# ksaintmarc/Montecarlo-PathTracing

Hardware: AMD Instinct MI355X
Metric: Msamples/s (W×H×spp/s) + achieved HBM GB/s, 1080p scene6, 1/2/4/8 GPU (higher is better)
Workload: dtype f32

## Files before the change

### montecarlo-pathtracing_amd/csrc/mcpt_capi.hip

```cpp
#include <algorithm>
#include <cmath>
#include <cstdio>
#include <cstring>
#include <new>

#include "mcpt_ctx.h"
#include "mcpt_math.h"

namespace plan = mcpt::plan;
static_assert(plan::kCandLane == MCPT_TRAVERSAL_LANE && plan::kCandWave == MCPT_TRAVERSAL_WAVE &&
              plan::kCandStream == MCPT_TRAVERSAL_STREAM, "candidates 1..3 are the traversal modes");

static thread_local char g_last_error[256] = "";
static thread_local char g_detail[320] = "";
static thread_local int g_last_status = 0;
static thread_local bool g_fresh = false;

int set_err(int status, const char* what, hipError_t e) {
  if (e != hipSuccess)
    std::snprintf(g_last_error, sizeof(g_last_error), "%s: %s", what, hipGetErrorString(e));
  else
    std::snprintf(g_last_error, sizeof(g_last_error), "%s", what);
  g_last_status = status;
  g_fresh = true;
// ... 822 lines not shown
  p.split_of = L.d_split_of;
  p.split_pass = L.d_split_pass;
  p.split_max = plan::kSplitMax;
  if (p.item_perm) p.split_n = L.d_split_n;
  if (steal) {
    OK_OR_RETURN(ensure_lane_bytes(c, L.d_steal, L.steal_bytes,
                                   sizeof(float) * 3 * (size_t)items * mcpt::kPassChunk * mcpt::kTileThreads));
    p.steal_vals = L.d_steal;
  }
  return MCPT_OK;
}

static int sort_order(mcpt_ctx* c, mcpt_ctx::Lane& L, hipStream_t ws, const plan::Items& it, const mcpt::RenderParams& p) {
  size_t tmp = L.sort_tmp_bytes;
  HIP_OR_RETURN(mcpt_order_items(L.d_item_cost, L.d_cost_sorted, L.d_item_iota, L.d_item_perm, (int)it.items,
                                 L.d_sort_tmp, &tmp, ws));
  if (c->n_meshes > 0)
    HIP_OR_RETURN(mcpt_split_count(L.d_cost_sorted, (int)it.items, 20 / (p.tile_w / 8) * c->n_cu, plan::kSplitMax,
                                   L.d_split_n, c->d_events + kDebugSplitSlot, ws));
  std::copy(it.key, it.key + 8, L.order_key);
  L.order_valid = true;
  L.order_age = 0;
  return MCPT_OK;
}

static int launch(mcpt_ctx* c, const float* invPV, const float* invV, int first_pass, int n_passes, float date,
                  int bounces, float refract_ind, int variant, bool count, unsigned long long* events) {
  OK_OR_RETURN(check_renderable(c, invPV && invV && n_passes >= 0 && variant >= 0 && variant <= 2, "mcpt_render"));
  invalidate_planes(c);
  HIP_OR_RETURN(hipSetDevice(c->device));
  mcpt::RenderParams p;
  scene_params(c, invPV, invV, p);
  plan::Tuner& tuner = c->tuner;
  HIP_OR_RETURN(collect_tuning(c, (tuner.pending_other_shape(p.n_local_px, n_passes) || count) ? 0 : 1));
  p.n_tiles = ((c->W + p.tile_w - 1) / p.tile_w) * ((c->n_local_rows + mcpt::kTileH - 1) / mcpt::kTileH);
  const long long total_seg = plan::pass_segments(first_pass, n_passes);
  tuner.deep_auto = c->depth >= 8;
  const int cand = count ? (c->traversal == MCPT_TRAVERSAL_AUTO ? MCPT_TRAVERSAL_LANE : c->traversal)
                         : resolve_candidate(c, total_seg);
  const bool stream = cand == plan::kCandStream && stream_applies(c, variant, bounces, count);
  c->stream_iters = 0;
  p.wave_traversal = (cand == MCPT_TRAVERSAL_WAVE) ? 1 : 0;
  p.walk_exit = plan::cand_walk_exit(cand, c->walk_exit, c->n_meshes, c->depth);
  p.leaf_batch = plan::cand_leaf_batch(cand, c->leaf_batch, c->depth);
  p.walk_min_done = plan::cand_deep_knobs(cand) ? plan::kDeepMinDone : 1;
  if (const int md = env_int("MCPT_WALK_MIN_DONE", 0); md > 0) p.walk_min_done = md;
  p.seg_per_item = plan::resolved_seg_per_item(cand, env_int("MCPT_SEG_PER_ITEM", 0));
  pass_params(first_pass, n_passes, date, bounces, refract_ind, variant, p);
  const bool steal = env_int("MCPT_STEAL", 1) != 0;
  plan::LimitsIn lin;
  lin.n_local_px = p.n_local_px; lin.n_tiles = p.n_tiles; lin.tile_w = p.tile_w; lin.seg_per_item = p.seg_per_item;
  lin.n_cu = c->n_cu; lin.partial_budget = c->partial_budget; lin.mesh = c->n_meshes > 0;
  lin.wave_traversal = p.wave_traversal != 0; lin.steal = steal;
  const plan::Limits lim = plan::limits(lin);
  if (lim.too_large) return set_err(MCPT_ERR_INVALID_ARG, "render target too large for one launch");
  const bool split = plan::pass_split(lim, p.n_tiles, n_passes, total_seg, c->n_cu, stream, env_int("MCPT_PASS_SPLIT", -1));
  p.pass_split = split ? 1 : 0;
  if (split) p.seg_per_item = 1;
  const int n_sub = plan::count_sub_launches(first_pass, n_passes, lim.max_seg, split);
  const size_t seg_bytes = (size_t)p.n_local_px * 3 * sizeof(float);
  const int slot = (c->ring_pos + 1) % kTimingRing;
  HIP_OR_RETURN(ensure_events(c, slot, std::max(n_sub, 1)));
  const bool lanes_ok = tuner.overlap != 0 && !count && !stream && schedule_settled(c);
  if (count) HIP_OR_RETURN(hipMemsetAsync(c->d_events, 0, sizeof(unsigned long long) * mcpt::EV_COUNT, c->stream));
  if (n_sub == 0) {
    for (int i = 0; i < kEvPerSub; ++i) HIP_OR_RETURN(hipEventRecord(ev_at(c, slot, 0, i), c->stream));
    c->ring_lane[slot][0] = 0;
  }
  plan::ItemsIn in;
  in.n_tiles = p.n_tiles; in.seg_per_item = p.seg_per_item; in.walk_exit = p.walk_exit; in.bounces = bounces;
  in.variant = variant; in.tile_w = p.tile_w; in.n_cu = c->n_cu; in.wave_traversal = p.wave_traversal != 0;
  in.pass_split = split; in.mesh = c->n_meshes > 0;
  in.orderable = !count && !stream && env_int("MCPT_ITEM_ORDER", 1) != 0;
  in.split_items_on = env_int("MCPT_SPLIT_ITEMS", 1) != 0;
  in.tail_pieces_on = env_int("MCPT_TAIL_PIECES", 1) != 0;
  int k = 0;
  for (long long lo = first_pass, end = (long long)first_pass + n_passes; lo < end; lo = in.sub.end(), ++k) {
    in.sub = plan::next_sub_launch(lo, end, lim.max_seg, split);
    const plan::Items it = plan::items(in);
    p.first_pass = in.sub.first_pass; p.n_passes = in.sub.n_passes; p.n_segments = in.sub.n_segments;
    p.item_perm = nullptr;
    p.item_cost = nullptr;
    p.split_n = nullptr; p.split_of = nullptr; p.split_pass = nullptr; p.split_max = 0;
    p.steal_vals = nullptr;
    p.n_items = (int)it.items;
    p.tail_m = 0;
#ifdef MCPT_CHECKED
    p.check_inject = env_int("MCPT_CHECKED_INJECT", 0);
#endif
    const int li = c->next_lane;
    c->next_lane ^= 1;
    mcpt_ctx::Lane& L = c->lanes[li];
    const bool lane = lanes_ok && p.n_segments > 1;
    hipStream_t ws = lane ? L.stream : c->stream;
    if (p.n_segments > 1) OK_OR_RETURN(ensure_lane_bytes(c, L.d_partial, L.partial_bytes, (size_t)p.n_segments * seg_bytes));
    p.partial = L.d_partial;
    if (it.order) HIP_OR_RETURN(ensure_item_order(c, L, it.items));
    if (lane) HIP_OR_RETURN(hipStreamWaitEvent(L.stream, lane_freed(c, L), 0));
    if (it.order) OK_OR_RETURN(prepare_order(c, li, ws, in, it, p));
    if (it.split_items) OK_OR_RETURN(prepare_split_items(c, L, ws, it.items, steal, p));
    const bool period = lane && c->prev_lane >= 0 && c->prev_lane != li;
    HIP_OR_RETURN(hipEventRecord(ev_at(c, slot, k, 0), period ? c->lanes[c->prev_lane].stream : ws));
    if (lane) HIP_OR_RETURN(hipEventRecord(ev_at(c, slot, k, 3), ws));
    c->ring_lane[slot][k] = lane;
    if (stream) {
      OK_OR_RETURN(stream_run(c, p));
    } else {
      HIP_OR_RETURN(mcpt_launch_render(p, count, ws));
    }
    HIP_OR_RETURN(hipEventRecord(ev_at(c, slot, k, 1), ws));
    if (lane) {
      HIP_OR_RETURN(hipStreamWaitEvent(c->stream, ev_at(c, slot, k, 1), 0));
      if (period) HIP_OR_RETURN(hipStreamWaitEvent(c->stream, ev_at(c, slot, k, 0), 0));
    }
    HIP_OR_RETURN(mcpt_launch_combine(p, c->stream));
    HIP_OR_RETURN(hipEventRecord(ev_at(c, slot, k, 2), c->stream));
    if (it.order && (!p.item_perm || ++L.order_age >= plan::kOrderRefresh)) OK_OR_RETURN(sort_order(c, L, ws, it, p));
    if (lane) {
      HIP_OR_RETURN(hipEventRecord(L.tail, L.stream));
      HIP_OR_RETURN(hipStreamWaitEvent(c->stream, L.tail, 0));
      HIP_OR_RETURN(hipEventRecord(L.freed, c->stream));
    }
    L.freed_stale = !lane;
    c->prev_lane = lane ? li : -1;
#ifdef MCPT_CHECKED
    OK_OR_RETURN(checked_sub_launch(c, k, n_sub, p));
#endif
  }
  if (!count && c->traversal == MCPT_TRAVERSAL_AUTO)
    tuner.issue(cand, (double)p.n_local_px * n_passes, p.n_local_px, n_passes, total_seg, slot);
  c->n_sub = std::max(n_sub, 1);
  c->ring_pos = slot;
  c->ring_n_sub[slot] = c->n_sub;
  c->n_timed++;
  c->pass_split = split ? 1 : 0;
  c->timed = true;
  c->pass_count += n_passes;
  if (c->ad_on && n_passes > 0)
    HIP_OR_RETURN(mcpt_launch_adaptive_add_passes(adaptive_target(c), nullptr, 0, n_passes, c->stream));
  if (c->stats_on && n_passes > 0) HIP_OR_RETURN(stats_batch(c, n_passes));
  if (count) {
    unsigned long long h[mcpt::EV_COUNT];
    HIP_OR_RETURN(hipMemcpyAsync(h, c->d_events, sizeof(h), hipMemcpyDeviceToHost, c->stream));
    HIP_OR_RETURN(hipStreamSynchronize(c->stream));
    for (int e = 0; e < mcpt::EV_COUNT; ++e) events[e] += h[e];
  }
  return MCPT_OK;
}

int mcpt_render(mcpt_ctx* c, const float* invPV, const float* invV, int first_pass, int n_passes, float date,
                int bounces, float refract_ind, int variant) {
  return launch(c, invPV, invV, first_pass, n_passes, date, bounces, refract_ind, variant, false, nullptr);
}
// ... 321 lines not shown
```

### montecarlo-pathtracing_amd/csrc/mcpt_internal.h

```cpp
#pragma once
#include <hip/hip_runtime.h>
#include <stdint.h>
#include "mcpt_plan.h"

int mcpt_err_bare(int status);

namespace mcpt {

enum { EV_NODE = 0, EV_LEAF, EV_PRIM, EV_CAND, EV_GEOM, EV_COLMAT, EV_SAMPLE, EV_TRAV, EV_MESH, EV_TRI, EV_MGEOM,
       EV_COUNT };

constexpr int kEventBytes[EV_COUNT] = {
    48,
    4,
    16 + 64,
    64,
    64,
    32,
    24,
    0,
    12 + 64 + 64,
    12 + 36,
    12 + 72 + 64,
};
// ... 194 lines not shown
                                hipStream_t stream);
hipError_t mcpt_launch_variance_init(const mcpt::CountSource* counts, const float* accum, float4* out,
                                     const float4* guide, const float2* emap, int W, int H, int pass_count,
                                     hipStream_t stream);
namespace mcpt {
struct TemporalParams {
  const float* accum;
  const float2* emap;
  const float4* guide;
  const float4* hc_in;
  const int* hl_in;
  const float4* hg_in;
  float4* hc_out;
  int* hl_out;
  float4* hg_out;
  unsigned long long* rec;
  int W, H;
  float nb;
  int max_history;
  float plane_tol;
  int empty;
  float M[16];
};
}
hipError_t mcpt_launch_temporal(const mcpt::TemporalParams& p, hipStream_t stream);
hipError_t mcpt_launch_temporal_init(const float4* hc, float4* out, const float4* guide, int W, int H,
                                     hipStream_t stream);
hipError_t mcpt_launch_pack_counted(const mcpt::CountSource& src, int n_rows, const float* accum, void* out,
                                    hipStream_t stream);
hipError_t mcpt_launch_load_rows_counted(const void* src, const int* src_row, int W, int H, float* accum, int* plane,
                                         hipStream_t stream);
hipError_t mcpt_launch_load_rows_error_map(const void* src, const int* src_row, int W, int H, float2* plane,
                                           hipStream_t stream);
hipError_t mcpt_iota(int* a, int n, hipStream_t stream);
hipError_t mcpt_split_count(const unsigned* cost_sorted, int n, int capacity, int split_max, int* out,
                            unsigned long long* dbg, hipStream_t stream);
constexpr int kDebugSplitSlot = 63;
constexpr int kDebugStealSlot = 62;

namespace mcpt {
constexpr int kCheckedCountSlot = 60, kCheckedSiteSlot = 61;
enum CheckSite {
  CK_SPLIT_N = 1,
  CK_PERM_SPLIT,
  CK_PERM_TAIL,
  CK_PERM_HEAD,
  CK_ITEM,
  CK_SPLIT_OF,
  CK_SPLIT_PASS,
  CK_SEGMENT,
  CK_PIXEL,
  CK_COMBINE_SPLIT,
  CK_LIST,
  CK_COUNT
};
#ifdef MCPT_CHECKED
constexpr bool kChecked = true;
__device__ inline bool idx_ok(unsigned long long* ev, int site, long long i, long long n) {
  if (i >= 0 && i < n) return true;
  if (ev) {
    atomicAdd(ev + kCheckedCountSlot, 1ull);
    atomicCAS(ev + kCheckedSiteSlot, 0ull, ((unsigned long long)site << 48) | ((unsigned long long)i & 0xffffffffffffull));
  }
  return false;
}
#else
constexpr bool kChecked = false;
__device__ __forceinline__ bool idx_ok(unsigned long long*, int, long long, long long) { return true; }
#endif
}
hipError_t mcpt_order_items(const unsigned* cost, unsigned* cost_sorted, const int* iota, int* perm, int n,
                            void* tmp, size_t* tmp_bytes, hipStream_t stream);
hipError_t mcpt_launch_stream_init(const mcpt::StreamParams& q, hipStream_t stream);
hipError_t mcpt_launch_stream_iter(const mcpt::StreamParams& q, int n_cu, bool lds_nodes, hipStream_t stream);
bool mcpt_stream_lds_nodes_fit(int depth);
```

### montecarlo-pathtracing_amd/csrc/mcpt_kernel.hip

```cpp
#include <hip/hip_runtime.h>
#include <stdint.h>
#include "mcpt_device.h"

constexpr int kMinWaves = 7;


namespace mcpt {

constexpr int kMinWavesMesh = 5;
constexpr int kMinWavesL2 = 7;
template <bool COUNT, bool WAVE, bool MESH, bool LDSS, bool SUSPEND, int TW, bool LIST = false>
__global__ __launch_bounds__(TW * kTileH, MESH && !WAVE ? kMinWavesMesh
                                           : (!WAVE && !LDSS ? kMinWavesL2 : kMinWaves)) void render_kernel(
    RenderParams p) {
  constexpr int TT = TW * kTileH;
  const int tid = threadIdx.x;
  const int lane = tid & 63, wave = tid >> 6;
  constexpr bool kSplit = MESH && !WAVE && !COUNT && !LIST;
  int item, piece = -1, sj = -1;
  if constexpr (kChecked) {
    if (p.check_inject) (void)idx_ok(p.events, CK_PERM_HEAD, blockIdx.x, p.n_items);
  }
  if constexpr (kSplit) {
    const int b = blockIdx.x;
    int sn = (p.item_perm && p.split_n) ? *p.split_n : 0;
    if (!idx_ok(p.events, CK_SPLIT_N, sn, (long long)p.split_max + 1)) sn = 0;
    if (b < sn * kSplitPieces) {
      sj = b / kSplitPieces;
      piece = b - sj * kSplitPieces;
      if (!idx_ok(p.events, CK_PERM_SPLIT, sj, p.n_items)) return;
      item = p.item_perm[sj];
    } else {
      const int r = sn + (b - sn * kSplitPieces);
      if (r >= p.n_items) return;
      item = p.item_perm ? p.item_perm[r] : r;
    }
  }
  int seg_only = -1;
  if constexpr (!kSplit) {
    const int b = blockIdx.x;
    const int head = p.tail_m > 0 ? p.n_items - p.tail_m : p.n_items;
    if (b >= head && p.tail_m > 0) {
      const int q = b - head, j = q / p.seg_per_item;
      if (!idx_ok(p.events, CK_PERM_TAIL, head + j, p.n_items)) return;
      item = p.item_perm[head + j];
      seg_only = q - j * p.seg_per_item;
    } else {
      if (!idx_ok(p.events, CK_PERM_HEAD, b, p.n_items)) return;
      item = p.item_perm ? p.item_perm[b] : b;
    }
  }
  if (!idx_ok(p.events, CK_ITEM, item, p.n_items)) return;
  const unsigned long long t_item0 = __builtin_amdgcn_s_memrealtime();
#ifdef MCPT_BLOCKTIMES
  const unsigned long long bt0 = __builtin_amdgcn_s_memrealtime();
#endif

  const int K = p.seg_per_item > 1 ? p.seg_per_item : 1;
  const int n_groups = (p.n_segments + K - 1) / K;
  const int tile = item / n_groups;
  int seg_lo = (item % n_groups) * K;
  int seg_n = min(K, p.n_segments - seg_lo);
  if (seg_only >= 0) {
    if (seg_only >= seg_n) return;
    seg_lo += seg_only;
    seg_n = 1;
  }
  int seg = seg_lo;
  const int tiles_x = (p.W + TW - 1) / TW;
  int bx0 = (tile % tiles_x) * TW + (wave % (TW / 8)) * 8;
  int by0 = (tile / tiles_x) * kTileH + (wave / (TW / 8)) * 8;
  bool listed = true;
  if constexpr (LIST) {
    static_assert(!COUNT && !WAVE, "LIST: the per-lane render kernels only");
    const long long li = (long long)tile * (TW / 8) + wave;
    int n_list = p.n_list;
    if (n_list < 0) {
      n_list = min(max(p.list[p.n_blocks], 0), -n_list);
      if ((long long)tile * (TW / 8) >= n_list) return;
    }
    listed = li < n_list && idx_ok(p.events, CK_LIST, li, p.n_blocks);
    const int blk = listed ? p.list[li] : 0;
    listed = listed && idx_ok(p.events, CK_LIST, blk, p.n_blocks);
    bx0 = (blk % p.blocks_x) * 8;
    by0 = (blk / p.blocks_x) * 8;
  }
  const int x = bx0 + (lane & 7);
  const int lr = by0 + (lane >> 3);
  const bool live = x < p.W && lr < p.n_local_rows && listed;
  const int cbase = floordiv(p.first_pass - 1, kPassChunk);
  const int c0 = cbase + seg_lo;
  int pass_begin = max(p.first_pass, c0 * kPassChunk + 1);
  int pass_end = min(p.first_pass + p.n_passes, (c0 + 1) * kPassChunk + 1);
  if (p.pass_split) {
    pass_begin = p.first_pass + seg_lo;
    pass_end = pass_begin + 1;
  }
  const int seg_first = pass_begin;
  int b1 = 0;
  if (kSplit && piece >= 0) {
    const int n = pass_end - pass_begin;
    b1 = pass_begin + n / kSplitPieces;
    const int lo = pass_begin + (piece * n) / kSplitPieces, hi = pass_begin + ((piece + 1) * n) / kSplitPieces;
    pass_begin = lo;
    pass_end = hi;
    if (piece == 0 && tid == 0 && idx_ok(p.events, CK_SPLIT_OF, item, p.n_items)) p.split_of[item] = sj;
  }
  const int y = live ? p.rows[lr] : 0;

  SceneT<MESH, LDSS> s{p.nodes, p.leaves, p.ptype, p.prims, p.depth, p.minfo, p.mpairs, p.mleaftris, p.mtris,
                       p.mverts, p.mnorms, p.flat_face};
  if constexpr (LDSS) {
    extern __shared__ float4 s_scene[];
    const int n_nodes = (2 << p.depth) - 1, n_leaves = 1 << p.depth;
    const int n4 = 3 * n_nodes + 8 * p.n_prims;
    for (int i = tid; i < n4; i += TT) s_scene[i] = i < 3 * n_nodes ? p.nodes[i] : p.prims[i - 3 * n_nodes];
    int* s_int = (int*)(s_scene + n4);
    for (int i = tid; i < n_leaves + p.n_prims; i += TT)
      s_int[i] = i < n_leaves ? p.leaves[i] : p.ptype[i - n_leaves];
    __syncthreads();
    s.nodes = s_scene;
    s.prims = s_scene + 3 * n_nodes;
    s.leaves = s_int;
    s.ptype = s_int + n_leaves;
  }
  static_assert(!kSplit || TT == 64, "pass stealing: one wave per workgroup (LDS order, unit mapping)");
  const bool steal = kSplit && p.steal_vals != nullptr;
  __shared__ int s_claim;
  __shared__ unsigned s_stolen;
  if constexpr (kSplit) {
    if (steal) {
      if (tid == 0) { s_claim = TT; s_stolen = 0u; }
      __syncthreads();
    }
  }
  Ev<COUNT> ev;
  ev.init();
#ifdef MCPT_LANESTATS
  for (int k = lane; k < LS_COUNT; k += 64) ls_row()[k] = 0u;
  __builtin_amdgcn_wave_barrier();
  if (!live) return;
#else
  if (!live) return;
#endif

  const float u = ((float)x + 0.5f) / (float)p.W;
  const float v = ((float)y + 0.5f) / (float)p.H;
  constexpr bool kPixLds = !LDSS || (MESH && !WAVE);
  constexpr bool kPxLds = kPixLds && MESH;
  constexpr bool kIorConst = kPixLds;
  __shared__ float s_pix[kPxLds ? 21 : (kPixLds ? 20 : 18)][TT];
  __shared__ int s_hit0[TT];
  const f3 Dcam0 = camera_dir(p, u, v);
  s_pix[0][tid] = Dcam0.x; s_pix[1][tid] = Dcam0.y; s_pix[2][tid] = Dcam0.z;
  if constexpr (kPixLds) {
    s_pix[18][tid] = u; s_pix[19][tid] = v;
    if constexpr (kPxLds) s_pix[20][tid] = __int_as_float(lr * p.W + x);
  }
  int pj = tid;
  auto pix_seed = [&](int ps) {
    if constexpr (kPixLds) return seed_for(s_pix[18][pj], s_pix[19][pj], ps, p.date);
    else return seed_for(((float)x + 0.5f) / (float)p.W, ((float)y + 0.5f) / (float)p.H, ps, p.date);
  };
  s_pix[12][tid] = 0.0f; s_pix[13][tid] = 0.0f; s_pix[14][tid] = 0.0f;
  const f3 Ocam = mk(p.ox, p.oy, p.oz);


  const float ior = p.ior;
  const int B = p.bounces;
  int pass = pass_begin;
  Rng rng = seed_for(u, v, pass, p.date);
  f3 O = Ocam, D = Dcam0, att = mk(0.8f, 0.8f, 0.8f), total = mk(0.0f, 0.0f, 0.0f);
  f3 N = mk(0.0f, 0.0f, 0.0f), P = mk(0.0f, 0.0f, 0.0f);
  int bounce = 0, phase = 0;
  Hit h;
  h.pl = mk(0.0f, 0.0f, 0.0f); h.dist = kFLTMAX; h.clear(); h.tri = 0;
  h.cull2 = 0.0;

  int key0 = -1;
  f3 N0 = N, P0 = P;
  const bool run = !(p.variant == 0 && B <= 0);
#ifdef MCPT_STAMPS
  unsigned long long st_k0 = __builtin_amdgcn_s_memtime(), st_t = 0, st_s = 0, st_it = 0;
#endif
  if (!COUNT && run) {
    traverse<COUNT, WAVE, SUSPEND && !LDSS && !MESH>(s, Ocam, Dcam0, h, ev);
    key0 = hit_key(h);
    if (h.hit()) geom_info<COUNT>(s, h, N0, P0, ev);
  }
  s_pix[3][tid] = N0.x; s_pix[4][tid] = N0.y; s_pix[5][tid] = N0.z;
  s_pix[6][tid] = P0.x; s_pix[7][tid] = P0.y; s_pix[8][tid] = P0.z;
  s_hit0[tid] = key0;

#ifdef MCPT_STAMPS
  const unsigned long long st_p = __builtin_amdgcn_s_memtime() - st_k0;
#endif
  auto flush_sum = [&]() {
    if (kSplit && (piece > 0 || steal)) return;
    size_t px;
    if constexpr (kPxLds) {
      px = (size_t)(unsigned)__float_as_int(s_pix[20][tid]);
    } else {
      int lrow = lr, col = x;
      asm volatile("" : "+v"(lrow), "+v"(col));
      px = (size_t)lrow * p.W + col;
    }
    if (!idx_ok(p.events, CK_PIXEL, (long long)px, p.n_local_px)) return;
    if (p.n_segments == 1) {
      float* accp = p.accum + px * 3;
      accp[0] = accp[0] + s_pix[12][tid]; accp[1] = accp[1] + s_pix[13][tid]; accp[2] = accp[2] + s_pix[14][tid];
    } else {
      if (!idx_ok(p.events, CK_SEGMENT, seg, p.n_segments)) return;
      float* part = p.partial + ((size_t)seg * p.n_local_px + px) * 3;
      part[0] = s_pix[12][tid]; part[1] = s_pix[13][tid]; part[2] = s_pix[14][tid];
    }
  };
  auto add_pass = [&](f3 v) {
    if (kSplit && steal) {
      if constexpr (kChecked) {
        if (!idx_ok(p.events, CK_SPLIT_PASS, pass - seg_first, kPassChunk) || !idx_ok(p.events, CK_SPLIT_PASS, pj, kTileThreads))
          return;
      }
      float* q = p.steal_vals + (((size_t)item * kPassChunk + (pass - seg_first)) * kTileThreads + pj) * 3;
      q[0] = v.x; q[1] = v.y; q[2] = v.z;
      return;
    }
    if (kSplit && piece > 0) {
      if constexpr (kChecked) {
        if (!idx_ok(p.events, CK_SPLIT_PASS, sj, p.split_max) || !idx_ok(p.events, CK_SPLIT_PASS, pass - b1, kPassChunk) ||
            !idx_ok(p.events, CK_SPLIT_PASS, tid, kTileThreads))
          return;
      }
      float* q = p.split_pass + (((size_t)sj * kPassChunk + (pass - b1)) * kTileThreads + tid) * 3;
      q[0] = v.x; q[1] = v.y; q[2] = v.z;
    } else {
      s_pix[12][tid] = s_pix[12][tid] + v.x;
      s_pix[13][tid] = s_pix[13][tid] + v.y;
      s_pix[14][tid] = s_pix[14][tid] + v.z;
    }
  };
  const int steal_n = pass_end - pass_begin;
  auto steal_next = [&]() {
    for (;;) {
      const int u = atomicAdd(&s_claim, 1);
      if (u >= TT * steal_n) { pass = pass_end; return; }
      const int t = u % TT;
      const int xt = bx0 + (t & 7), lt = by0 + (t >> 3);
      if (xt < p.W && lt < p.n_local_rows) {
        pj = t; pass = pass_begin + u / TT;
        if (t != tid) atomicAdd(&s_stolen, 1u);
        return;
      }
    }
  };
  auto next_chunk = [&]() {
    if (kSplit && steal) {
      steal_next();
      return;
    }
    if (pass >= pass_end) {
      flush_sum();
      if (seg + 1 < seg_lo + seg_n) {
        seg++;
        const int c = c0 + (seg - seg_lo);
        pass = c * kPassChunk + 1;
        pass_end = min(p.first_pass + p.n_passes, (c + 1) * kPassChunk + 1);
        s_pix[12][tid] = 0.0f; s_pix[13][tid] = 0.0f; s_pix[14][tid] = 0.0f;
      }
    }
  };
  Walk walk;
  walk.invD = mk(0.0f, 0.0f, 0.0f); walk.node = 0; walk.level = 0; walk.pending = 0; walk.mpf = 0;
  bool walking = false;
#ifdef MCPT_LANESTATS
  ls_add(LS_WAVES, 1u);
#endif
  while (pass < pass_end) {
#ifdef MCPT_STAMPS
    const unsigned long long st_a = __builtin_amdgcn_s_memtime();
    st_it++;
#endif
#ifdef MCPT_LANESTATS
    ls_add(LS_ROUNDS, 1u);
    ls_add(LS_ROUND_LN, ls_pop(true));
#endif
    bool done = false;
    f3 res = mk(0.0f, 0.0f, 0.0f);
    bool first = !COUNT && bounce == 0 && phase == 0;
    bool ready = true;
    if (!run) {
      done = true;
    } else {
      if (first) {
        h.code = s_hit0[pj];
      } else if (WAVE) {
        traverse<COUNT, WAVE>(s, O, D, h, ev);
      } else {
        if (!walking) { walk_begin<COUNT>(s, D, h, walk, ev, p.cull2_max); walking = true; }
        if constexpr (MESH) {
          walking = !walk_run_mesh<COUNT, SUSPEND>(s, O, D, h, walk, ev, p.walk_exit);
        } else {
          walking = !walk_run<COUNT, SUSPEND>(s, O, D, h, walk, ev, p.walk_exit, p.leaf_batch, p.walk_min_done);
        }
        ready = !walking;
      }
    }
#ifdef MCPT_STAMPS
    const unsigned long long st_b = __builtin_amdgcn_s_memtime();
// ... 135 lines not shown
          P = mk(s_pix[15][tid], s_pix[16][tid], s_pix[17][tid]);
        }
        O = add(P, muls(N, kBIAS));
        D = grefract(D, neg(N), p.inv_ior, kIorConst ? p.inv_ior_sq : p.inv_ior * p.inv_ior);
        phase = 0;
        bounce++;
        if (bounce >= B) done = true;
      }
    }
    if (done) {
      add_pass(res);
      ev.inc(EV_SAMPLE);
      pass++;
      next_chunk();
      rng = pix_seed(pass);
      O = Ocam; D = mk(s_pix[0][pj], s_pix[1][pj], s_pix[2][pj]);
      att = mk(0.8f, 0.8f, 0.8f); total = mk(0.0f, 0.0f, 0.0f);
      bounce = 0; phase = 0;
    }
#ifdef MCPT_STAMPS
    st_s += __builtin_amdgcn_s_memtime();
#endif
  }
#ifdef MCPT_STAMPS
  {
    unsigned long long vals[6] = {__builtin_amdgcn_s_memtime() - st_k0, st_p, st_t, st_s, st_it, ev.st_leaf};
    unsigned long long it_sum = st_it, lit = ev.st_lit, wit = ev.st_wit;
    unsigned long long nl = ev.st_nl, nw = ev.st_nw, ll = ev.st_ll, lw = ev.st_lw;
    for (int off = 32; off > 0; off >>= 1) {
      for (int k = 0; k < 6; ++k) { unsigned long long o = __shfl_xor(vals[k], off); vals[k] = vals[k] > o ? vals[k] : o; }
      it_sum += __shfl_xor(it_sum, off);
      lit += __shfl_xor(lit, off);
      wit += __shfl_xor(wit, off);
      nl += __shfl_xor(nl, off);
      nw += __shfl_xor(nw, off);
      ll += __shfl_xor(ll, off);
      lw += __shfl_xor(lw, off);
    }
    if ((int)__lane_id() == __builtin_ffsll((long long)__ballot(1)) - 1 && p.events) {
      for (int k = 0; k < 5; ++k) atomicAdd(p.events + k, vals[k]);
      atomicAdd(p.events + 5, it_sum);
      atomicAdd(p.events + 6, 1ull);
      atomicAdd(p.events + 7, vals[5]);
      atomicAdd(p.events + 9, lit);
      atomicAdd(p.events + 10, wit);
      atomicAdd(p.events + 11, nl);
      atomicAdd(p.events + 12, nw);
      atomicAdd(p.events + 13, ll);
      atomicAdd(p.events + 14, lw);
    }
  }
#endif

  if constexpr (kSplit) {
    if (steal && p.events && (int)__lane_id() == __builtin_ffsll((long long)__ballot(1)) - 1 && s_stolen)
      atomicAdd(p.events + kDebugStealSlot, (unsigned long long)s_stolen);
  }
  if (p.item_cost && (int)__lane_id() == __builtin_ffsll((long long)__ballot(1)) - 1) {
    unsigned long long dt = __builtin_amdgcn_s_memrealtime() - t_item0;
    if (kSplit && piece >= 0) dt *= kSplitPieces;
    if (seg_only >= 0) dt *= (unsigned)p.seg_per_item;
    atomicMax(p.item_cost + item, dt < 0xffffffffull ? (unsigned)dt : 0xffffffffu);
  }
#ifdef MCPT_BLOCKTIMES
  {
    const unsigned long long bt1 = __builtin_amdgcn_s_memrealtime();
    const int lead = __builtin_ffsll((long long)__ballot(1)) - 1, k = (int)__lane_id() - lead;
    const unsigned long long slot = 2ull * ((unsigned long long)blockIdx.x * (TT / 64) + wave) + k;
    if ((k == 0 || k == 1) && p.events && slot < kBlockTimeSlots)
      p.events[kBlockTimeBase + slot] = k ? bt1 : bt0;
  }
#endif
#ifdef MCPT_LANESTATS
  if (ls_lead() && p.events)
    for (int k = 0; k < LS_COUNT; ++k) atomicAdd(p.events + 16 + k, (unsigned long long)ls_row()[k]);
#endif
  if (COUNT) {
#pragma unroll
    for (int e = 0; e < EV_COUNT; ++e) {
      unsigned long long vsum = ev.c.v[e];
      for (int off = 32; off > 0; off >>= 1) vsum += __shfl_xor(vsum, off);
      if (lane == 0) atomicAdd(p.events + e, vsum);
    }
  }
}

__global__ __launch_bounds__(256) void combine_split_kernel(float* __restrict__ accum, const float* __restrict__ partial,
                                                            long long n_px, int first_pass, int n_passes) {
  long long i = (long long)blockIdx.x * 256 + threadIdx.x;
  if (i >= n_px) return;
  float a0 = accum[i * 3], a1 = accum[i * 3 + 1], a2 = accum[i * 3 + 2];
  float s0 = 0.0f, s1 = 0.0f, s2 = 0.0f;
  for (int k = 0; k < n_passes; ++k) {
    const float* q = partial + ((size_t)k * n_px + i) * 3;
    s0 = s0 + q[0]; s1 = s1 + q[1]; s2 = s2 + q[2];
    const int pass = first_pass + k;
    if (k + 1 == n_passes || floordiv(pass - 1, kPassChunk) != floordiv(pass, kPassChunk)) {
      a0 = a0 + s0; a1 = a1 + s1; a2 = a2 + s2;
      s0 = 0.0f; s1 = 0.0f; s2 = 0.0f;
    }
  }
  accum[i * 3] = a0; accum[i * 3 + 1] = a1; accum[i * 3 + 2] = a2;
}

__global__ __launch_bounds__(256) void combine_kernel(float* __restrict__ accum, const float* __restrict__ partial,
                                                      long long n_px, int n_seg) {
// ... 6 lines not shown
  }
  accum[i * 3] = a0; accum[i * 3 + 1] = a1; accum[i * 3 + 2] = a2;
}

__global__ __launch_bounds__(256) void combine_items_kernel(float* __restrict__ accum, const float* __restrict__ partial,
                                                            long long n_px, int n_seg, int W, int TW,
                                                            const int* __restrict__ split_of,
                                                            const float* __restrict__ split_pass, int split_max,
                                                            unsigned long long* ev) {
  long long i = (long long)blockIdx.x * 256 + threadIdx.x;
  if (i >= n_px) return;
  const int lr = (int)(i / W), x = (int)(i - (long long)lr * W);
  const int tiles_x = (W + TW - 1) / TW;
  const int tile = (lr / kTileH) * tiles_x + x / TW;
  const int t = (((lr % kTileH) / 8) * (TW / 8) + (x % TW) / 8) * 64 + (lr % 8) * 8 + (x % 8);
  constexpr int p1 = kPassChunk / kSplitPieces;
  float a0 = accum[i * 3], a1 = accum[i * 3 + 1], a2 = accum[i * 3 + 2];
  for (int s = 0; s < n_seg; ++s) {
    const float* q = partial + ((size_t)s * n_px + i) * 3;
    float s0 = q[0], s1 = q[1], s2 = q[2];
    const int j = split_of[(size_t)tile * n_seg + s];
    if (j >= 0 && idx_ok(ev, CK_COMBINE_SPLIT, j, split_max)) {
      for (int k = 0; k < kPassChunk - p1; ++k) {
        const float* v = split_pass + (((size_t)j * kPassChunk + k) * kTileThreads + t) * 3;
        s0 = s0 + v[0]; s1 = s1 + v[1]; s2 = s2 + v[2];
      }
    }
    a0 = a0 + s0; a1 = a1 + s1; a2 = a2 + s2;
  }
  accum[i * 3] = a0; accum[i * 3 + 1] = a1; accum[i * 3 + 2] = a2;
}

__global__ __launch_bounds__(256) void combine_steal_kernel(float* __restrict__ accum, long long n_px, int n_seg,
                                                            int W, int TW, const float* __restrict__ vals) {
  long long i = (long long)blockIdx.x * 256 + threadIdx.x;
  if (i >= n_px) return;
  const int lr = (int)(i / W), x = (int)(i - (long long)lr * W);
  const int tiles_x = (W + TW - 1) / TW;
  const int tile = (lr / kTileH) * tiles_x + x / TW;
  const int t = (((lr % kTileH) / 8) * (TW / 8) + (x % TW) / 8) * 64 + (lr % 8) * 8 + (x % 8);
  float a0 = accum[i * 3], a1 = accum[i * 3 + 1], a2 = accum[i * 3 + 2];
  for (int s = 0; s < n_seg; ++s) {
    const size_t item = (size_t)tile * n_seg + s;
    float s0 = 0.0f, s1 = 0.0f, s2 = 0.0f;
    for (int k = 0; k < kPassChunk; ++k) {
      const float* v = vals + ((item * kPassChunk + k) * kTileThreads + t) * 3;
      s0 = s0 + v[0]; s1 = s1 + v[1]; s2 = s2 + v[2];
    }
    a0 = a0 + s0; a1 = a1 + s1; a2 = a2 + s2;
  }
  accum[i * 3] = a0; accum[i * 3 + 1] = a1; accum[i * 3 + 2] = a2;
}

template <bool ANY, bool MESH>
__global__ __launch_bounds__(256) void trace_kernel(TraceParams q) {
  const long long i = (long long)blockIdx.x * 256 + threadIdx.x;
  if (i >= q.n) return;
  SceneT<MESH> s{q.nodes, q.leaves, q.ptype, q.prims, q.depth, q.minfo, q.mpairs, q.mleaftris, q.mtris, q.mverts,
                 q.mnorms, q.flat_face};
  Ev<false> ev;
  const f3 O = mk(q.orig[3 * i], q.orig[3 * i + 1], q.orig[3 * i + 2]);
  const f3 D = mk(q.dir[3 * i], q.dir[3 * i + 1], q.dir[3 * i + 2]);
  Hit h;
  h.pl = mk(0.0f, 0.0f, 0.0f); h.cull2 = 0.0;
  if (q.prim < 0) {
    traverse_lane<false, ANY>(s, O, D, h, ev);
  } else {
    h.clear(); h.dist = kFLTMAX; h.cull2 = cull_bound_sq(kFLTMAX);
    prim_test<false, false, ANY>(s, q.prim, O, D, h, ev);
  }
  float* o = q.out + i * kTraceFloats;
  int* oi = q.out_i + i * 3;
  oi[0] = h.hit() ? h.shape() : -1;
  oi[1] = h.hit() ? h.index() : -1;
  oi[2] = !h.hit() ? -1 : (h.shape() == CODE_MESH ? h.tri : h.face());
  f3 N = mk(0.0f, 0.0f, 0.0f), P = N;
  float4 col = make_float4(0.0f, 0.0f, 0.0f, 0.0f), mat = col;
  f3 pg = h.pl;
  if (h.hit()) {
    const size_t b = (size_t)h.index() * 8;
    pg = xpoint(s.prims[b + 3], s.prims[b + 4], s.prims[b + 5], h.pl);
    geom_info<false>(s, h, N, P, ev);
    col = s.prims[(size_t)h.index() * 8 + 6];
    mat = s.prims[(size_t)h.index() * 8 + 7];
  }
  const float v[kTraceFloats] = {h.hit() ? h.dist : kFLTMAX, h.pl.x, h.pl.y, h.pl.z, pg.x, pg.y, pg.z,
                                 N.x, N.y, N.z, P.x, P.y, P.z, col.x, col.y, col.z, col.w, mat.x, mat.y, mat.z, mat.w};
#pragma unroll
  for (int k = 0; k < kTraceFloats; ++k) o[k] = v[k];
}

__global__ __launch_bounds__(256) void sample_kernel(SampleParams q) {
  const long long k = (long long)blockIdx.x * 256 + threadIdx.x;
  if (k >= q.n) return;
  const uint32_t step = (uint32_t)k * q.nb_used;
  Rng rng;
  rng.x = fbits(q.fseed[0]) + step * 11u;
  rng.y = fbits(q.fseed[1]) + step * 43u;
  rng.z = fbits(q.fseed[2]) + step * 67u;
  const f3 n = normalize3(mk(q.normal[0], q.normal[1], q.normal[2]));
  const f3 r = random_ray(rng, n, q.roughness);
  q.out[3 * k] = r.x; q.out[3 * k + 1] = r.y; q.out[3 * k + 2] = r.z;
}

}


hipError_t mcpt_launch_trace(const mcpt::TraceParams& q, bool any_hit, hipStream_t stream) {
  if (q.n <= 0) return hipSuccess;
  dim3 block(256), grid((unsigned)((q.n + 255) / 256));
  if (q.n_meshes > 0) {
    if (any_hit) hipLaunchKernelGGL((mcpt::trace_kernel<true, true>), grid, block, 0, stream, q);
    else hipLaunchKernelGGL((mcpt::trace_kernel<false, true>), grid, block, 0, stream, q);
  } else {
    if (any_hit) hipLaunchKernelGGL((mcpt::trace_kernel<true, false>), grid, block, 0, stream, q);
    else hipLaunchKernelGGL((mcpt::trace_kernel<false, false>), grid, block, 0, stream, q);
  }
  return hipGetLastError();
}

hipError_t mcpt_launch_sample(const mcpt::SampleParams& q, hipStream_t stream) {
  if (q.n <= 0) return hipSuccess;
  dim3 block(256), grid((unsigned)((q.n + 255) / 256));
  hipLaunchKernelGGL(mcpt::sample_kernel, grid, block, 0, stream, q);
  return hipGetLastError();
}

hipError_t mcpt_launch_render(const mcpt::RenderParams& p, bool count, hipStream_t stream) {
  const int K = p.seg_per_item > 1 ? p.seg_per_item : 1;
  const long long items = (long long)p.n_tiles * ((p.n_segments + K - 1) / K);
  if (items <= 0) return hipSuccess;
  const long long blocks = items + (p.split_of ? (long long)p.split_max * (mcpt::kSplitPieces - 1) : 0) +
                           (long long)p.tail_m * (K - 1);
  dim3 block(p.tile_w * mcpt::kTileH), grid((unsigned)blocks);
  const bool wave = p.wave_traversal != 0, mesh = p.n_meshes > 0;
  const bool lds = p.lds_scene_bytes > 0;
  if (p.tile_w != mcpt::tile_w_for(mesh, p.lds_scene_bytes)) return hipErrorInvalidValue;
  const bool susp = !count && !wave && (p.walk_exit > 0 || p.leaf_batch > 0);
  const size_t shm = lds ? (size_t)p.lds_scene_bytes : 0;
#define MCPT_RENDER(C, W, M, L, S, T) \
  hipLaunchKernelGGL((mcpt::render_kernel<C, W, M, L, S, T>), grid, block, shm, stream, p)
#define MCPT_RENDER_CW(C, W, S)                                          \
  if (mesh && lds) MCPT_RENDER(C, W, true, true, S, 8);                  \
  else if (mesh) MCPT_RENDER(C, W, true, false, S, 8);                   \
  else if (lds && p.tile_w == 16) MCPT_RENDER(C, W, false, true, S, 16); \
  else if (lds) MCPT_RENDER(C, W, false, true, S, 32);                   \
  else MCPT_RENDER(C, W, false, false, S, 16)
  if (count) {
    if (wave) { MCPT_RENDER_CW(true, true, false); } else { MCPT_RENDER_CW(true, false, false); }
  } else if (wave) {
    MCPT_RENDER_CW(false, true, false);
  } else if (susp) {
    MCPT_RENDER_CW(false, false, true);
  } else {
    MCPT_RENDER_CW(false, false, false);
  }
#undef MCPT_RENDER_CW
#undef MCPT_RENDER
  return hipGetLastError();
}

hipError_t mcpt_launch_render_list(const mcpt::RenderParams& p, hipStream_t stream) {
  const long long items = (long long)p.n_tiles * p.n_segments;
  const long long held = p.n_list < 0 ? -(long long)p.n_list : p.n_list;
  if (items <= 0 || held <= 0) return hipSuccess;
  const bool mesh = p.n_meshes > 0, lds = p.lds_scene_bytes > 0;
  if (!p.list || p.wave_traversal || p.seg_per_item != 1 || p.pass_split || p.item_perm || p.tail_m || p.split_of ||
      p.steal_vals || p.n_items != items || p.tile_w != mcpt::tile_w_for(mesh, p.lds_scene_bytes) ||
      (long long)p.n_tiles * (p.tile_w / 8) < held)
    return hipErrorInvalidValue;
  dim3 block(p.tile_w * mcpt::kTileH), grid((unsigned)items);
  const size_t shm = lds ? (size_t)p.lds_scene_bytes : 0;
#define MCPT_RENDER_LIST(M, L, S, T) \
  hipLaunchKernelGGL((mcpt::render_kernel<false, false, M, L, S, T, true>), grid, block, shm, stream, p)
#define MCPT_RENDER_LIST_S(S)                                          \
  if (mesh && lds) MCPT_RENDER_LIST(true, true, S, 8);                 \
  else if (mesh) MCPT_RENDER_LIST(true, false, S, 8);                  \
  else if (lds && p.tile_w == 16) MCPT_RENDER_LIST(false, true, S, 16); \
  else if (lds) MCPT_RENDER_LIST(false, true, S, 32);                  \
  else MCPT_RENDER_LIST(false, false, S, 16)
  if (p.walk_exit > 0 || p.leaf_batch > 0) { MCPT_RENDER_LIST_S(true); } else { MCPT_RENDER_LIST_S(false); }
#undef MCPT_RENDER_LIST_S
#undef MCPT_RENDER_LIST
  return hipGetLastError();
}

hipError_t mcpt_launch_combine(const mcpt::RenderParams& p, hipStream_t stream) {
  if (p.n_local_px <= 0) return hipSuccess;
  dim3 block(256), grid((unsigned)((p.n_local_px + 255) / 256));
  if (p.steal_vals) {
    hipLaunchKernelGGL(mcpt::combine_steal_kernel, grid, block, 0, stream, p.accum, p.n_local_px, p.n_segments, p.W,
                       p.tile_w, p.steal_vals);
    return hipGetLastError();
  }
  if (p.n_segments <= 1) return hipSuccess;
  if (p.pass_split)
    hipLaunchKernelGGL(mcpt::combine_split_kernel, grid, block, 0, stream, p.accum, p.partial, p.n_local_px,
                       p.first_pass, p.n_passes);
  else if (p.split_of)
    hipLaunchKernelGGL(mcpt::combine_items_kernel, grid, block, 0, stream, p.accum, p.partial, p.n_local_px,
                       p.n_segments, p.W, p.tile_w, p.split_of, p.split_pass, p.split_max, p.events);
  else
    hipLaunchKernelGGL(mcpt::combine_kernel, grid, block, 0, stream, p.accum, p.partial, p.n_local_px, p.n_segments);
  return hipGetLastError();
}
```

### montecarlo-pathtracing_amd/csrc/mcpt_plan.h

```cpp
#pragma once
#include <stddef.h>

#include <algorithm>

namespace mcpt {

constexpr int kPassChunk = 32;
constexpr int kSplitPieces = 4;
constexpr int kTileW = 32, kTileH = 8;
constexpr int kTileThreads = kTileW * kTileH;

namespace plan {

constexpr size_t kDefaultPartialBudget = size_t(4) << 30;
constexpr size_t kStealBudget = size_t(8) << 30;
constexpr long long kOrderMinItems = 4096;
constexpr int kOrderRefresh = 16;
constexpr int kSplitMax = 1024;
constexpr int kPassSplitItemsPerCu = 4, kPassSplitMaxPasses = 256;

constexpr long long floor_div(long long a, long long b) { return (a >= 0) ? a / b : -((-a + b - 1) / b); }
constexpr long long pass_segments(long long first_pass, long long n_passes) {
  return n_passes > 0 ? floor_div(first_pass + n_passes - 2, kPassChunk) - floor_div(first_pass - 1, kPassChunk) + 1 : 0;
}

struct LimitsIn {
  long long n_local_px = 0, n_tiles = 0;
  int tile_w = 16, seg_per_item = 1, n_cu = 256;
  size_t partial_budget = kDefaultPartialBudget;
  bool mesh = false, wave_traversal = false;
  bool steal = true;
  bool spare = true;
};
struct Limits {
  long long max_items = 0;
  long long max_seg = 1;
  bool may_steal = false;
  bool too_large = false;
};
inline Limits limits(const LimitsIn& in) {
  Limits r;
  const long long seg_bytes = in.n_local_px * 3 * (long long)sizeof(float);
  const long long kseg_max = std::max(1, in.seg_per_item);
  const long long spare = in.spare ? (long long)kSplitMax * (kSplitPieces - 1) + 28LL * in.n_cu * (kseg_max - 1) : 0;
  r.max_items = (1LL << 32) / (in.tile_w * kTileH) - 1 - spare;
  r.too_large = in.n_tiles > r.max_items;
  long long max_seg = seg_bytes > 0 ? (long long)(in.partial_budget / (size_t)seg_bytes) : (1LL << 30);
  r.may_steal = in.mesh && !in.wave_traversal && kseg_max == 1 && in.steal;
  if (r.may_steal && seg_bytes > 0)
    max_seg = std::min(max_seg, std::max(2LL, (long long)(kStealBudget / ((size_t)seg_bytes * kPassChunk))));
  r.max_seg = std::max(1LL, std::min(max_seg, in.n_tiles > 0 ? r.max_items / in.n_tiles : r.max_items));
  return r;
}

inline bool pass_split(const Limits& lim, long long n_tiles, int n_passes, long long total_seg, int n_cu,
                       bool stream, int env_split) {
  const bool split_fits = !stream && n_passes > 1 && n_passes <= lim.max_seg && n_passes <= kPassSplitMaxPasses &&
                          n_tiles * (long long)n_passes <= lim.max_items;
  return split_fits && (env_split >= 0 ? env_split > 0 : n_tiles * total_seg < (long long)kPassSplitItemsPerCu * n_cu);
}

struct SubLaunch {
  int first_pass = 0, n_passes = 0, n_segments = 0;
  long long end() const { return (long long)first_pass + n_passes; }
};
inline SubLaunch next_sub_launch(long long lo, long long end, long long max_seg, bool split) {
  const long long c0 = floor_div(lo - 1, kPassChunk);
  const long long hi = split ? end : std::min(end, (c0 + max_seg) * kPassChunk + 1);
  SubLaunch s;
  s.first_pass = (int)lo;
  s.n_passes = (int)(hi - lo);
  s.n_segments = split ? s.n_passes : (int)(floor_div(hi - 2, kPassChunk) - c0 + 1);
  return s;
}
inline int count_sub_launches(long long first_pass, long long n_passes, long long max_seg, bool split) {
  int n = 0;
  for (long long lo = first_pass, end = first_pass + n_passes; lo < end; ++n)
    lo = next_sub_launch(lo, end, max_seg, split).end();
  return n;
}

struct ItemsIn {
  long long n_tiles = 0;
  SubLaunch sub;
  int seg_per_item = 1, walk_exit = 0, bounces = 0, variant = 0, tile_w = 16, n_cu = 256;
  bool wave_traversal = false, pass_split = false, mesh = false;
  bool orderable = true;
  bool split_items_on = true;
  bool tail_pieces_on = true;
};
struct Items {
  int kseg = 1;
  long long items = 0;
  long long key[8] = {};
  bool order = false;
  bool split_items = false;
};
inline Items items(const ItemsIn& in) {
  Items r;
  r.kseg = in.seg_per_item > 1 ? in.seg_per_item : 1;
  r.items = in.n_tiles * ((in.sub.n_segments + r.kseg - 1) / r.kseg);
  const long long key[8] = {r.items, in.sub.n_segments, r.kseg, in.wave_traversal, in.walk_exit, in.bounces,
                            in.variant, (long long)in.pass_split};
// ... 154 lines not shown
```

Before: 15110.

## Add intra-wave work stealing for LDS-scene render kernels with per-pass value buffer

Adds a STEAL variant of the LDS-scene (non-mesh) render kernel. Lanes within a wave claim (pixel, pass) units from a shared LDS counter, so idle lanes take over work from slow lanes instead of waiting on divergence. Each pass result is written to a large per-tile, per-pass global buffer, and a new combine kernel reduces these buffers into the accumulator. This trades wave divergence idle time for much more HBM write and read traffic, a buffer of up to 16 GiB, and atomics on LDS.

```diff
diff --git a/montecarlo-pathtracing_amd/csrc/mcpt_capi.hip b/montecarlo-pathtracing_amd/csrc/mcpt_capi.hip
--- a/montecarlo-pathtracing_amd/csrc/mcpt_capi.hip
+++ b/montecarlo-pathtracing_amd/csrc/mcpt_capi.hip
@@ -898,6 +898,9 @@
   lin.n_local_px = p.n_local_px; lin.n_tiles = p.n_tiles; lin.tile_w = p.tile_w; lin.seg_per_item = p.seg_per_item;
   lin.n_cu = c->n_cu; lin.partial_budget = c->partial_budget; lin.mesh = c->n_meshes > 0;
   lin.wave_traversal = p.wave_traversal != 0; lin.steal = steal;
+  const bool scene_steal = steal && p.lds_scene_bytes > 0 && c->n_meshes == 0 && !p.wave_traversal && !count &&
+                           !stream && schedule_settled(c);
+  lin.lds_scene = scene_steal;
   const plan::Limits lim = plan::limits(lin);
   if (lim.too_large) return set_err(MCPT_ERR_INVALID_ARG, "render target too large for one launch");
   const bool split = plan::pass_split(lim, p.n_tiles, n_passes, total_seg, c->n_cu, stream, env_int("MCPT_PASS_SPLIT", -1));
@@ -945,6 +948,11 @@
     if (lane) HIP_OR_RETURN(hipStreamWaitEvent(L.stream, lane_freed(c, L), 0));
     if (it.order) OK_OR_RETURN(prepare_order(c, li, ws, in, it, p));
     if (it.split_items) OK_OR_RETURN(prepare_split_items(c, L, ws, it.items, steal, p));
+    if (scene_steal && lim.may_steal && p.n_segments > 1 && !split) {
+      OK_OR_RETURN(ensure_lane_bytes(c, L.d_steal, L.steal_bytes, sizeof(float) * 3 * (size_t)p.n_tiles * p.n_segments *
+                                                                      mcpt::kPassChunk * p.tile_w * mcpt::kTileH));
+      p.steal_vals = L.d_steal;
+    }
     const bool period = lane && c->prev_lane >= 0 && c->prev_lane != li;
     HIP_OR_RETURN(hipEventRecord(ev_at(c, slot, k, 0), period ? c->lanes[c->prev_lane].stream : ws));
     if (lane) HIP_OR_RETURN(hipEventRecord(ev_at(c, slot, k, 3), ws));
diff --git a/montecarlo-pathtracing_amd/csrc/mcpt_internal.h b/montecarlo-pathtracing_amd/csrc/mcpt_internal.h
--- a/montecarlo-pathtracing_amd/csrc/mcpt_internal.h
+++ b/montecarlo-pathtracing_amd/csrc/mcpt_internal.h
@@ -270,6 +270,7 @@
   CK_PIXEL,
   CK_COMBINE_SPLIT,
   CK_LIST,
+  CK_STEAL_SLOT,
   CK_COUNT
 };
 #ifdef MCPT_CHECKED
diff --git a/montecarlo-pathtracing_amd/csrc/mcpt_kernel.hip b/montecarlo-pathtracing_amd/csrc/mcpt_kernel.hip
--- a/montecarlo-pathtracing_amd/csrc/mcpt_kernel.hip
+++ b/montecarlo-pathtracing_amd/csrc/mcpt_kernel.hip
@@ -9,7 +9,7 @@
 
 constexpr int kMinWavesMesh = 5;
 constexpr int kMinWavesL2 = 7;
-template <bool COUNT, bool WAVE, bool MESH, bool LDSS, bool SUSPEND, int TW, bool LIST = false>
+template <bool COUNT, bool WAVE, bool MESH, bool LDSS, bool SUSPEND, int TW, bool LIST = false, bool STEAL = false>
 __global__ __launch_bounds__(TW * kTileH, MESH && !WAVE ? kMinWavesMesh
                                            : (!WAVE && !LDSS ? kMinWavesL2 : kMinWaves)) void render_kernel(
     RenderParams p) {
@@ -17,6 +17,7 @@
   const int tid = threadIdx.x;
   const int lane = tid & 63, wave = tid >> 6;
   constexpr bool kSplit = MESH && !WAVE && !COUNT && !LIST;
+  static_assert(!STEAL || (LDSS && !MESH && !WAVE && !COUNT && !LIST), "STEAL: the LDS-scene render kernels");
   int item, piece = -1, sj = -1;
   if constexpr (kChecked) {
     if (p.check_inject) (void)idx_ok(p.events, CK_PERM_HEAD, blockIdx.x, p.n_items);
@@ -97,6 +98,7 @@
     pass_end = pass_begin + 1;
   }
   const int seg_first = pass_begin;
+  if constexpr (STEAL) pass_end = min(p.first_pass + p.n_passes, (c0 + seg_n) * kPassChunk + 1);
   int b1 = 0;
   if (kSplit && piece >= 0) {
     const int n = pass_end - pass_begin;
@@ -108,6 +110,8 @@
   }
   const int y = live ? p.rows[lr] : 0;
 
+  __shared__ int s_wclaim[STEAL ? TT / 64 : 1];
+  __shared__ unsigned s_wstolen[STEAL ? TT / 64 : 1];
   SceneT<MESH, LDSS> s{p.nodes, p.leaves, p.ptype, p.prims, p.depth, p.minfo, p.mpairs, p.mleaftris, p.mtris,
                        p.mverts, p.mnorms, p.flat_face};
   if constexpr (LDSS) {
@@ -118,6 +122,9 @@
     int* s_int = (int*)(s_scene + n4);
     for (int i = tid; i < n_leaves + p.n_prims; i += TT)
       s_int[i] = i < n_leaves ? p.leaves[i] : p.ptype[i - n_leaves];
+    if constexpr (STEAL) {
+      if (lane == 0) { s_wclaim[wave] = 64; s_wstolen[wave] = 0u; }
+    }
     __syncthreads();
     s.nodes = s_scene;
     s.prims = s_scene + 3 * n_nodes;
@@ -160,9 +167,14 @@
   int pj = tid;
   auto pix_seed = [&](int ps) {
     if constexpr (kPixLds) return seed_for(s_pix[18][pj], s_pix[19][pj], ps, p.date);
+    else if constexpr (STEAL) return seed_for(s_pix[12][pj], s_pix[13][pj], ps, p.date);
     else return seed_for(((float)x + 0.5f) / (float)p.W, ((float)y + 0.5f) / (float)p.H, ps, p.date);
   };
-  s_pix[12][tid] = 0.0f; s_pix[13][tid] = 0.0f; s_pix[14][tid] = 0.0f;
+  if constexpr (STEAL) {
+    s_pix[12][tid] = u; s_pix[13][tid] = v;
+  } else {
+    s_pix[12][tid] = 0.0f; s_pix[13][tid] = 0.0f; s_pix[14][tid] = 0.0f;
+  }
   const f3 Ocam = mk(p.ox, p.oy, p.oz);
 
 
@@ -196,6 +208,7 @@
   const unsigned long long st_p = __builtin_amdgcn_s_memtime() - st_k0;
 #endif
   auto flush_sum = [&]() {
+    if constexpr (STEAL) return;
     if (kSplit && (piece > 0 || steal)) return;
     size_t px;
     if constexpr (kPxLds) {
@@ -216,6 +229,18 @@
     }
   };
   auto add_pass = [&](f3 v) {
+    if constexpr (STEAL) {
+      const int ch = (pass - 1) >> 5, sg = ch - cbase, off = (pass - 1) & (kPassChunk - 1);
+      if constexpr (kChecked) {
+        if (!idx_ok(p.events, CK_STEAL_SLOT, sg, p.n_segments) || !idx_ok(p.events, CK_STEAL_SLOT, pj, TT) ||
+            !idx_ok(p.events, CK_STEAL_SLOT, tile, p.n_tiles))
+          return;
+      }
+      const unsigned slot = (((unsigned)(tile * p.n_segments + sg) * kPassChunk + off) * TT + (unsigned)pj);
+      float* q = p.steal_vals + (size_t)slot * 3;
+      q[0] = v.x; q[1] = v.y; q[2] = v.z;
+      return;
+    }
     if (kSplit && steal) {
       if constexpr (kChecked) {
         if (!idx_ok(p.events, CK_SPLIT_PASS, pass - seg_first, kPassChunk) || !idx_ok(p.events, CK_SPLIT_PASS, pj, kTileThreads))
@@ -253,7 +278,24 @@
       }
     }
   };
+  auto wave_steal_next = [&]() {
+    const int n_units = 64 * (pass_end - pass_begin);
+    for (;;) {
+      const int u = atomicAdd(&s_wclaim[STEAL ? wave : 0], 1);
+      if (u >= n_units) { pass = pass_end; return; }
+      const int t = u & 63;
+      if (bx0 + (t & 7) < p.W && by0 + (t >> 3) < p.n_local_rows) {
+        pj = wave * 64 + t; pass = pass_begin + (u >> 6);
+        if (t != lane) atomicAdd(&s_wstolen[STEAL ? wave : 0], 1u);
+        return;
+      }
+    }
+  };
   auto next_chunk = [&]() {
+    if constexpr (STEAL) {
+      wave_steal_next();
+      return;
+    }
     if (kSplit && steal) {
       steal_next();
       return;
@@ -495,6 +537,10 @@
   }
 #endif
 
+  if constexpr (STEAL) {
+    if (p.events && (int)__lane_id() == __builtin_ffsll((long long)__ballot(1)) - 1 && s_wstolen[wave])
+      atomicAdd(p.events + kDebugStealSlot, (unsigned long long)s_wstolen[wave]);
+  }
   if constexpr (kSplit) {
     if (steal && p.events && (int)__lane_id() == __builtin_ffsll((long long)__ballot(1)) - 1 && s_stolen)
       atomicAdd(p.events + kDebugStealSlot, (unsigned long long)s_stolen);
@@ -607,6 +653,35 @@
   accum[i * 3] = a0; accum[i * 3 + 1] = a1; accum[i * 3 + 2] = a2;
 }
 
+__global__ __launch_bounds__(256) void combine_steal_seg_kernel(float* __restrict__ accum, int n_tiles, int n_seg, int W,
+                                                                int n_local_rows, int TW, const float* __restrict__ vals,
+                                                                int first_pass, int n_passes, unsigned long long* ev) {
+  const int TT = TW * kTileH;
+  const long long g = (long long)blockIdx.x * 256 + threadIdx.x;
+  if (g >= (long long)n_tiles * TT) return;
+  const int tile = (int)(g / TT), t = (int)(g - (long long)tile * TT);
+  const int tiles_x = (W + TW - 1) / TW, wv = t >> 6, l = t & 63;
+  const int x = (tile % tiles_x) * TW + (wv % (TW / 8)) * 8 + (l & 7);
+  const int lr = (tile / tiles_x) * kTileH + (wv / (TW / 8)) * 8 + (l >> 3);
+  if (x >= W || lr >= n_local_rows) return;
+  const long long i = (long long)lr * W + x;
+  if (!idx_ok(ev, CK_PIXEL, i, (long long)n_local_rows * W)) return;
+  const int cbase = floordiv(first_pass - 1, kPassChunk);
+  float a0 = accum[i * 3], a1 = accum[i * 3 + 1], a2 = accum[i * 3 + 2];
+  for (int s = 0; s < n_seg; ++s) {
+    const int c = cbase + s;
+    const int lo = max(first_pass, c * kPassChunk + 1), hi = min(first_pass + n_passes, (c + 1) * kPassChunk + 1);
+    const float* row = vals + ((((size_t)tile * n_seg + s) * kPassChunk) * TT + t) * 3;
+    float s0 = 0.0f, s1 = 0.0f, s2 = 0.0f;
+    for (int ps = lo; ps < hi; ++ps) {
+      const float* v = row + (size_t)(ps - (c * kPassChunk + 1)) * TT * 3;
+      s0 = s0 + v[0]; s1 = s1 + v[1]; s2 = s2 + v[2];
+    }
+    a0 = a0 + s0; a1 = a1 + s1; a2 = a2 + s2;
+  }
+  accum[i * 3] = a0; accum[i * 3 + 1] = a1; accum[i * 3 + 2] = a2;
+}
+
 template <bool ANY, bool MESH>
 __global__ __launch_bounds__(256) void trace_kernel(TraceParams q) {
   const long long i = (long long)blockIdx.x * 256 + threadIdx.x;
@@ -695,6 +770,17 @@
   const size_t shm = lds ? (size_t)p.lds_scene_bytes : 0;
 #define MCPT_RENDER(C, W, M, L, S, T) \
   hipLaunchKernelGGL((mcpt::render_kernel<C, W, M, L, S, T>), grid, block, shm, stream, p)
+  if (p.steal_vals && !mesh) {
+    if (!lds || count || wave || p.pass_split || p.n_segments < 2) return hipErrorInvalidValue;
+    if (p.tile_w == 16) {
+      if (susp) hipLaunchKernelGGL((mcpt::render_kernel<false, false, false, true, true, 16, false, true>), grid, block, shm, stream, p);
+      else hipLaunchKernelGGL((mcpt::render_kernel<false, false, false, true, false, 16, false, true>), grid, block, shm, stream, p);
+    } else {
+      if (susp) hipLaunchKernelGGL((mcpt::render_kernel<false, false, false, true, true, 32, false, true>), grid, block, shm, stream, p);
+      else hipLaunchKernelGGL((mcpt::render_kernel<false, false, false, true, false, 32, false, true>), grid, block, shm, stream, p);
+    }
+    return hipGetLastError();
+  }
 #define MCPT_RENDER_CW(C, W, S)                                          \
   if (mesh && lds) MCPT_RENDER(C, W, true, true, S, 8);                  \
   else if (mesh) MCPT_RENDER(C, W, true, false, S, 8);                   \
@@ -743,6 +829,13 @@
 hipError_t mcpt_launch_combine(const mcpt::RenderParams& p, hipStream_t stream) {
   if (p.n_local_px <= 0) return hipSuccess;
   dim3 block(256), grid((unsigned)((p.n_local_px + 255) / 256));
+  if (p.steal_vals && p.n_meshes == 0) {
+    const long long n_thr = (long long)p.n_tiles * p.tile_w * mcpt::kTileH;
+    hipLaunchKernelGGL(mcpt::combine_steal_seg_kernel, dim3((unsigned)((n_thr + 255) / 256)), block, 0, stream, p.accum,
+                       p.n_tiles, p.n_segments, p.W, p.n_local_rows, p.tile_w, p.steal_vals, p.first_pass, p.n_passes,
+                       p.events);
+    return hipGetLastError();
+  }
   if (p.steal_vals) {
     hipLaunchKernelGGL(mcpt::combine_steal_kernel, grid, block, 0, stream, p.accum, p.n_local_px, p.n_segments, p.W,
                        p.tile_w, p.steal_vals);
diff --git a/montecarlo-pathtracing_amd/csrc/mcpt_plan.h b/montecarlo-pathtracing_amd/csrc/mcpt_plan.h
--- a/montecarlo-pathtracing_amd/csrc/mcpt_plan.h
+++ b/montecarlo-pathtracing_amd/csrc/mcpt_plan.h
@@ -14,6 +14,7 @@
 
 constexpr size_t kDefaultPartialBudget = size_t(4) << 30;
 constexpr size_t kStealBudget = size_t(8) << 30;
+constexpr size_t kSceneStealBudget = size_t(16) << 30;
 constexpr long long kOrderMinItems = 4096;
 constexpr int kOrderRefresh = 16;
 constexpr int kSplitMax = 1024;
@@ -29,6 +30,7 @@
   int tile_w = 16, seg_per_item = 1, n_cu = 256;
   size_t partial_budget = kDefaultPartialBudget;
   bool mesh = false, wave_traversal = false;
+  bool lds_scene = false;
   bool steal = true;
   bool spare = true;
 };
@@ -49,6 +51,15 @@
   r.may_steal = in.mesh && !in.wave_traversal && kseg_max == 1 && in.steal;
   if (r.may_steal && seg_bytes > 0)
     max_seg = std::min(max_seg, std::max(2LL, (long long)(kStealBudget / ((size_t)seg_bytes * kPassChunk))));
+  if (in.lds_scene && !in.mesh && !in.wave_traversal && in.steal) {
+    r.may_steal = true;
+    const long long val_bytes = in.n_tiles * in.tile_w * kTileH * 3 * (long long)sizeof(float) * kPassChunk;
+    if (val_bytes * kseg_max >= (12LL << 32)) r.may_steal = false;
+    else if (val_bytes > 0) {
+      const long long fit = (long long)(kSceneStealBudget / (size_t)val_bytes);
+      max_seg = std::min(max_seg, std::max(kseg_max, fit / kseg_max * kseg_max));
+    }
+  }
   r.max_seg = std::max(1LL, std::min(max_seg, in.n_tiles > 0 ? r.max_items / in.n_tiles : r.max_items));
   return r;
 }
```

New measurement: 15620 (median of 6 runs). 3.4% higher.
